# apache/spark

Measured on AMD Instinct MI355X. Metric: rows/sec (sort+hash-agg+join, 1B-row synth), higher is better.
Workload: dtype int64; 1 GPU; orderby-1b-int64x3 (BASELINE configs[1]); value = sort rows/s; rows=1000000000, cols=int64 key + int64 + float64 payload, parallelism=single GPU

## Files before the change

### spark_amd/csrc/gpuq.hip

```cpp
#include <hip/hip_runtime.h>
#include <stdint.h>
#include <stdio.h>
#include <string.h>

#include "../../include/gpuq.h"


static __thread char g_err[512];

extern "C" const char* gpuq_last_error(void) { return g_err; }

#define FAIL(code, ...) do { \
    snprintf(g_err, sizeof(g_err), __VA_ARGS__); return (code); } while (0)

#define HIP_TRY(expr) do { hipError_t _e = (expr); if (_e != hipSuccess) { \
    snprintf(g_err, sizeof(g_err), "%s failed: %s (%s:%d)", #expr, \
             hipGetErrorString(_e), __FILE__, __LINE__); \
    return GPUQ_ERR_HIP; } } while (0)

extern "C" int gpuq_device_count(void) {
  int n = 0;
  if (hipGetDeviceCount(&n) != hipSuccess) return 0;
  return n;
}
// ... 61 lines not shown
  h1 ^= k1; h1 = rotl32(h1, 13); return h1 * 5u + 0xe6546b64u;
}
DEV uint32_t mm3_fmix(uint32_t h1, uint32_t len) {
  h1 ^= len; h1 ^= h1 >> 16; h1 *= 0x85ebca6bu; h1 ^= h1 >> 13;
  h1 *= 0xc2b2ae35u; h1 ^= h1 >> 16; return h1;
}
DEV int32_t mm3_hash_long(int64_t input, int32_t seed) {
  uint32_t lo = (uint32_t)(uint64_t)input;
  uint32_t hi = (uint32_t)((uint64_t)input >> 32);
  uint32_t h1 = mm3_mixH1((uint32_t)seed, mm3_mixK1(lo));
  h1 = mm3_mixH1(h1, mm3_mixK1(hi));
  return (int32_t)mm3_fmix(h1, 8);
}
DEV int32_t spark_pmod(int32_t a, int32_t n) {
  int32_t r = a % n; return r < 0 ? r + n : r;
}

DEV uint64_t splitmix64(uint64_t x) {
  x += 0x9E3779B97F4A7C15ULL;
  x = (x ^ (x >> 30)) * 0xBF58476D1CE4E5B9ULL;
  x = (x ^ (x >> 27)) * 0x94D049BB133111EBULL;
  return x ^ (x >> 31);
}
DEV uint64_t gen_u64_dev(uint64_t seed, uint64_t i) {
  return splitmix64(seed * 0x9E3779B97F4A7C15ULL + i);
}

#define SIGNBIT 0x8000000000000000ULL

DEV uint64_t encode_f64(double v) {
  if (v == -0.0) v = 0.0;
  uint64_t bits;
  if (v != v) bits = 0x7ff8000000000000ULL;
  else bits = __double_as_longlong(v);
  uint64_t mask = (uint64_t)(-(int64_t)(bits >> 63)) | SIGNBIT;
  return bits ^ mask;
}
DEV uint64_t encode_i64(int64_t v) { return (uint64_t)v ^ SIGNBIT; }

DEV int64_t decode_i64(uint64_t e) { return (int64_t)(e ^ SIGNBIT); }
DEV double decode_f64(uint64_t e) {
  uint64_t mask = ((e >> 63) ? 0 : ~0ULL) | SIGNBIT;
  return __longlong_as_double((long long)(e ^ mask));
}

DEV uint64_t sort_out_word(uint64_t kk, int decode_mode) {
  if (!decode_mode) return kk;
  uint64_t e = (decode_mode & 4) ? ~kk : kk;
  if (decode_mode & 2) {
    uint64_t mask = ((e >> 63) ? 0 : ~0ULL) | SIGNBIT;
    return e ^ mask;
  }
  return e ^ SIGNBIT;
}

DEV bool bit_valid(const uint8_t* validity, int64_t i) {
  return !validity || ((validity[i >> 3] >> (i & 7)) & 1);
}


__global__ void k_gen_i64_range(uint64_t seed, uint64_t start, int64_t n,
                                uint64_t range, int64_t* out) {
  int64_t i = (int64_t)blockIdx.x * blockDim.x + threadIdx.x;
  int64_t stride = (int64_t)gridDim.x * blockDim.x;
  for (; i < n; i += stride) {
    uint64_t v = gen_u64_dev(seed, start + (uint64_t)i);
    out[i] = (int64_t)(range ? v % range : v);
  }
}

__global__ void k_gen_f64_unit(uint64_t seed, uint64_t start, int64_t n, double* out) {
  int64_t i = (int64_t)blockIdx.x * blockDim.x + threadIdx.x;
  int64_t stride = (int64_t)gridDim.x * blockDim.x;
  for (; i < n; i += stride) {
    uint64_t v = gen_u64_dev(seed, start + (uint64_t)i);
    out[i] = (double)(v >> 11) * (1.0 / 9007199254740992.0);
  }
}

static dim3 hash_grid(int64_t n, int block = 256) {
  static int cap = -2;
  if (cap == -2) {
    const char* e = getenv("GPUQ_HASH_GRID");
    cap = e ? atoi(e) : 2048;
  }
  int64_t b = (n + block - 1) / block;
  if (cap > 0 && b > cap) b = cap;
  if (b > 0x7FFFFFFF) b = 0x7FFFFFFF;
  if (b < 1) b = 1;
  return dim3((uint32_t)b);
}

static dim3 grid1d(int64_t n, int block = 256) {
  int64_t b = (n + block - 1) / block;
  if (b > 2048) b = 2048;
  if (b < 1) b = 1;
  return dim3((uint32_t)b);
}

extern "C" int gpuq_gen_i64_range(void* stream, uint64_t seed, uint64_t start,
                                  int64_t n, uint64_t range, int64_t* out) {
  k_gen_i64_range<<<grid1d(n), 256, 0, (hipStream_t)stream>>>(seed, start, n, range, out);
  HIP_TRY(hipGetLastError());
  return GPUQ_OK;
}

// ... 135 lines not shown
  if (n == 0) return GPUQ_OK;
  { hipEvent_t _pe = prof_begin(s);
  k_interleave2<<<grid1d(n), 256, 0, s>>>(n, (const uint64_t*)a,
                                          (const uint64_t*)b,
                                          (ulonglong2*)scratch);
  prof_end("interleave2", s, _pe); }
  HIP_TRY(hipGetLastError());
  static int mlp = -1;
  if (mlp < 0) mlp = getenv("GPUQ_GATHER_MLP") ? atoi(getenv("GPUQ_GATHER_MLP")) : 0;
  { hipEvent_t _pe = prof_begin(s);
  if (mlp)
    k_gather2_pairs4<<<grid1d((n + 3) / 4), 256, 0, s>>>(
        n, (const ulonglong2*)scratch, perm, (uint64_t*)oa, (uint64_t*)ob);
  else
    k_gather2_pairs<<<grid1d(n), 256, 0, s>>>(n, (const ulonglong2*)scratch,
                                              perm, (uint64_t*)oa,
                                              (uint64_t*)ob);
  prof_end("gather2_pairs", s, _pe); }
  HIP_TRY(hipGetLastError());
  return GPUQ_OK;
}

extern "C" int gpuq_gather(void* stream, int64_t n, gpuq_col col,
                           const uint32_t* perm, void* out) {
  hipStream_t s = (hipStream_t)stream;
  if (col.dtype == GPUQ_INT64 || col.dtype == GPUQ_FLOAT64) {
    k_gather<uint64_t><<<grid1d(n, 256), 256, 0, s>>>(n, (const uint64_t*)col.data, perm, (uint64_t*)out);
  } else if (col.dtype == GPUQ_INT32) {
    k_gather<uint32_t><<<grid1d(n, 256), 256, 0, s>>>(n, (const uint32_t*)col.data, perm, (uint32_t*)out);
  } else {
    FAIL(GPUQ_ERR_INVALID, "gather: unsupported dtype %d", col.dtype);
  }
  HIP_TRY(hipGetLastError());
  return GPUQ_OK;
}


#define SORT_BLOCK 256
#define SORT_WAVES (SORT_BLOCK / WAVE)
#define SORT_ITEMS 16
#define SORT_TILE (SORT_BLOCK * SORT_ITEMS)

template <int DTYPE, bool DESC>
__global__ void k_encode(int64_t n, const void* keys, const uint32_t* rowmap,
                         uint64_t* ek, uint32_t* idx,
                         unsigned long long* bits_and, unsigned long long* bits_or,
                         uint32_t* ghist ) {
  __shared__ uint32_t h[8][256];
  for (int b = threadIdx.x; b < 8 * 256; b += blockDim.x) ((uint32_t*)h)[b] = 0;
  __syncthreads();
  uint64_t acc_or = 0, acc_and = ~0ULL;
  int64_t i = (int64_t)blockIdx.x * blockDim.x + threadIdx.x;
  int64_t stride = (int64_t)gridDim.x * blockDim.x;
  for (; i < n; i += stride) {
    uint64_t e;
    uint32_t row = rowmap ? rowmap[i] : (uint32_t)i;
    if (DTYPE == GPUQ_FLOAT64) e = encode_f64(((const double*)keys)[row]);
    else e = encode_i64(((const int64_t*)keys)[row]);
    if (DESC) e = ~e;
    ek[i] = e;
    idx[i] = row;
    acc_or |= e; acc_and &= e;
    #pragma unroll
    for (int b = 0; b < 8; b++) atomicAdd(&h[b][(e >> (b * 8)) & 0xff], 1u);
  }
  for (int off = 32; off > 0; off >>= 1) {
    acc_or |= __shfl_down((unsigned long long)acc_or, off);
    acc_and &= __shfl_down((unsigned long long)acc_and, off);
  }
  if ((threadIdx.x & (WAVE - 1)) == 0) {
    atomicOr(bits_or, (unsigned long long)acc_or);
    atomicAnd(bits_and, (unsigned long long)acc_and);
  }
  __syncthreads();
  for (int b = threadIdx.x; b < 8 * 256; b += blockDim.x) {
    uint32_t v = ((uint32_t*)h)[b];
    if (v) atomicAdd(&ghist[b], v);
  }
}

struct scatter_geom { int block, items; };
static scatter_geom get_sort_geom(void);

template <int BIN_MODE>
DEV int compute_bin(uint64_t key, int shift, int nparts) {
  (void)nparts;
  if (BIN_MODE == 0) return (int)((key >> shift) & 0xff);
  if (BIN_MODE == 2)
    return (int)(((uint32_t)mm3_hash_long((int64_t)key, 42)) >> 24);
  return (int)((((uint32_t)mm3_hash_long((int64_t)key, 42)) >> (16 + shift)) & 0xff);
}

__global__ void k_validity_pids(int64_t n, const uint8_t* validity, int nulls_first,
                                uint64_t* pid_as_key, uint32_t* idx,
                                unsigned long long* null_count) {
  __shared__ unsigned int h;
  if (threadIdx.x == 0) h = 0;
  __syncthreads();
  int64_t i = (int64_t)blockIdx.x * blockDim.x + threadIdx.x;
  int64_t stride = (int64_t)gridDim.x * blockDim.x;
  unsigned int mine = 0;
  for (; i < n; i += stride) {
    bool valid = (validity[i >> 3] >> (i & 7)) & 1;
    pid_as_key[i] = (uint64_t)(valid == (bool)nulls_first);
    idx[i] = (uint32_t)i;
    if (!valid) mine++;
  }
  if (mine) atomicAdd(&h, mine);
  __syncthreads();
  if (threadIdx.x == 0 && h) atomicAdd(null_count, (unsigned long long)h);
}

template <int BIN_MODE>
__global__ void k_radix_hist(int64_t n, const uint64_t* keys, int shift,
// ... 65 lines not shown
    __syncthreads();
    if (threadIdx.x == 0) {
      uint32_t acc = 0;
      for (int w = 0; w < SCAN_BLOCK / WAVE; w++) { uint32_t t = wsum[w]; wsum[w] = acc; acc += t; }
      carry_s = acc;
    }
    __syncthreads();
    if (i < n) sums[i] = s - v + wsum[wave] + carry;
    carry += carry_s;
    __syncthreads();
  }
}

__global__ void k_scan_add(int64_t n, const uint32_t* in, uint32_t* out,
                           const uint32_t* block_sums) {
  int64_t base = (int64_t)blockIdx.x * SCAN_TILE;
  uint32_t add = block_sums[blockIdx.x];
  for (int r = 0; r < SCAN_ITEMS; r++) {
    int64_t i = base + r * SCAN_BLOCK + threadIdx.x;
    if (i < n) out[i] = out[i] - in[i] + add;
  }
}

static int exclusive_scan_u32(hipStream_t s, int64_t n, const uint32_t* in,
                              uint32_t* out, uint32_t* block_sums ) {
  int64_t nblocks = (n + SCAN_TILE - 1) / SCAN_TILE;
  k_scan_partial<<<dim3((uint32_t)nblocks), SCAN_BLOCK, 0, s>>>(n, in, out, block_sums);
  k_scan_sums<<<1, SCAN_BLOCK, 0, s>>>(nblocks, block_sums);
  k_scan_add<<<dim3((uint32_t)nblocks), SCAN_BLOCK, 0, s>>>(n, in, out, block_sums);
  HIP_TRY(hipGetLastError());
  return GPUQ_OK;
}

#define OSW_AGG (1ULL << 54)
#define OSW_PFX (2ULL << 54)
#define OSW_VAL(x) ((x) & ((1ULL << 54) - 1))
#define OSW_EPOCH(x) ((x) >> 56)
#define OSW_SPIN_LIMIT (1u << 22)

typedef unsigned long long ull2_a8 __attribute__((vector_size(16), aligned(8)));
typedef uint32_t u32v2_a4 __attribute__((vector_size(8), aligned(4)));

template <int BIN_MODE, int BLOCK, int ITEMS, bool LOOKBACK, typename PayT = uint32_t,
          int RADIX_BITS = 8, bool CONTIG = false>
__global__ __launch_bounds__(BLOCK)
void k_radix_scatter(int64_t n, const uint64_t* kin, const PayT* iin,
                     uint64_t* kout, PayT* iout,
                     const uint32_t* scanned ,
                     int shift, int nblocks, int nparts,
                     unsigned long long* state ,
                     const uint32_t* gbase ,
                     unsigned long long* err_flag, uint32_t epoch,
                     void* decode_out ,
                     int decode_mode ) {
  constexpr int WAVES = BLOCK / WAVE;
  constexpr int TILE = BLOCK * ITEMS;
  constexpr int BINS = 1 << RADIX_BITS;
  __shared__ uint32_t wave_hist[WAVES][BINS];
  __shared__ uint32_t bin_start[BINS];
  __shared__ uint32_t bin_gbase[BINS];
  __shared__ uint32_t wtot[WAVES <= 4 ? 4 : WAVES];
  __shared__ uint32_t bin_cnt[(LOOKBACK && RADIX_BITS < 8) ? BINS : 1];
  __shared__ uint64_t stage_k[TILE];
  __shared__ PayT stage_i[TILE];

  const int tid = threadIdx.x;
  const int wave = tid / WAVE, lane = tid & (WAVE - 1);
  const int64_t base = (int64_t)blockIdx.x * TILE;
  const int tile_n = (int)min((int64_t)TILE, n - base);

  for (int b = tid; b < WAVES * BINS; b += BLOCK)
    ((uint32_t*)wave_hist)[b] = 0;
  __syncthreads();

  uint64_t k[ITEMS];
  PayT id[ITEMS];
  uint16_t lrank[ITEMS];
  uint8_t lbin[ITEMS];

  const int64_t wbase = base + (int64_t)wave * WAVE * ITEMS;
  #pragma unroll
  for (int r = 0; r < ITEMS; r++) {
    int64_t i = wbase + r * WAVE + lane;
    bool valid = i < n;
    k[r] = valid ? kin[i] : 0;
    id[r] = valid ? iin[i] : 0;
  }
  for (int r = 0; r < ITEMS; r++) {
    int64_t i = wbase + r * WAVE + lane;
    bool valid = i < n;
    int bin = valid ? compute_bin<BIN_MODE>(k[r], shift, nparts) : 0;
    if (RADIX_BITS < 8) bin &= (1 << RADIX_BITS) - 1;
    lbin[r] = (uint8_t)bin;
    uint64_t active = __ballot(valid);
    uint64_t same = active;
    for (int b = 0; b < RADIX_BITS; b++) {
      uint64_t bl = __ballot((bin >> b) & 1);
      same &= ((bin >> b) & 1) ? bl : ~bl;
    }
    uint64_t below = same & ((1ULL << lane) - 1);
    int rank = __popcll(below);
    int leader = __ffsll((unsigned long long)same) - 1;
    uint32_t basecnt = 0;
    if (valid && lane == leader) {
      basecnt = wave_hist[wave][bin];
      wave_hist[wave][bin] = basecnt + __popcll(same);
    }
    basecnt = __shfl(basecnt, leader);
    lrank[r] = (uint16_t)(basecnt + rank);
    __builtin_amdgcn_wave_barrier();
  }
  __syncthreads();

  uint32_t acc = 0;
  if (tid < BINS) {
    int bin = tid;
    for (int w = 0; w < WAVES; w++) {
      uint32_t t = wave_hist[w][bin];
      wave_hist[w][bin] = acc;
      acc += t;
    }
    if (LOOKBACK) {
      __hip_atomic_store(&state[(int64_t)blockIdx.x * 256 + bin],
                         ((unsigned long long)epoch << 56) | OSW_AGG | acc,
                         __ATOMIC_RELAXED, __HIP_MEMORY_SCOPE_AGENT);
      if (RADIX_BITS < 8) bin_cnt[bin] = acc;
    }
    uint32_t inc = wave_inclusive_scan(acc);
    if (lane == WAVE - 1) wtot[wave] = inc;
    bin_start[bin] = inc - acc;
  }
  __syncthreads();
  if (tid < BINS) {
    int bin = tid;
    uint32_t woff = 0;
    for (int w = 0; w < wave; w++) woff += wtot[w];
    uint32_t excl = bin_start[bin] + woff;
    bin_start[bin] = excl;
    if (!LOOKBACK) {
// ... 152 lines not shown
    if (j < tile_n) {
      uint64_t kk = stage_k[j];
      int bin = compute_bin<BIN_MODE>(kk, shift, nparts);
      if (RADIX_BITS < 8) bin &= (1 << RADIX_BITS) - 1;
      uint32_t dst = bin_gbase[bin] + (uint32_t)j;
      uint64_t kv_out = sort_out_word(kk, decode_mode);
      void* kdst = decode_mode ? (void*)&((uint64_t*)decode_out)[dst]
                               : (void*)&kout[dst];
#ifdef GPUQ_DRAIN_SC1
      __hip_atomic_store((uint64_t*)kdst, kv_out, __ATOMIC_RELAXED,
                         __HIP_MEMORY_SCOPE_AGENT);
      __hip_atomic_store((PayT*)&iout[dst], stage_i[j], __ATOMIC_RELAXED,
                         __HIP_MEMORY_SCOPE_AGENT);
#elif defined(GPUQ_DRAIN_NT)
      __builtin_nontemporal_store(kv_out, (uint64_t*)kdst);
      __builtin_nontemporal_store(stage_i[j], &iout[dst]);
#else
      *(uint64_t*)kdst = kv_out;
      iout[dst] = stage_i[j];
#endif
    }
  }
}

static scatter_geom get_sort_geom(void) {
  static scatter_geom g = {0, 0};
  if (g.block == 0) {
    const char* e = getenv("GPUQ_SORT_GEOM");
    int b = 0, it = 0;
    if (e && sscanf(e, "%dx%d", &b, &it) == 2) { g.block = b; g.items = it; }
    else { g.block = 256; g.items = 22; }
    static const int known[][2] = {{256,16},{512,8},{512,16},{1024,8},{512,4},
                                   {512,6},{256,12},{512,12},{1024,5},{512,10},
                                   {1024,2},{1024,6},{1024,4},{512,11},
                                   {256,20},{256,22}};
    bool ok = false;
    for (auto& k : known) ok = ok || (k[0] == g.block && k[1] == g.items);
    if (!ok) {
      fprintf(stderr, "gpuq: unsupported GPUQ_SORT_GEOM %dx%d, using 256x22\n",
              g.block, g.items);
      g.block = 256; g.items = 22;
    }
  }
  return g;
}

template <int BIN_MODE, bool LOOKBACK>
static void launch_scatter(hipStream_t s, scatter_geom g, int64_t nb,
                           int64_t n, const uint64_t* kin, const uint32_t* iin,
                           uint64_t* kout, uint32_t* iout,
                           const uint32_t* scanned, int shift, int nparts,
                           unsigned long long* state, const uint32_t* gbase,
                           unsigned long long* err_flag, uint32_t epoch,
                           void* decode_out = nullptr, int decode_mode = 0) {
  dim3 grid((uint32_t)nb);
#define LS(B, I) k_radix_scatter<BIN_MODE, B, I, LOOKBACK><<<grid, B, 0, s>>>( \
      n, kin, iin, kout, iout, scanned, shift, (int)nb, nparts, state, gbase, \
      err_flag, epoch, decode_out, decode_mode)
  static int contig = -1;
  if (contig < 0) contig = getenv("GPUQ_DRAIN_CONTIG") != nullptr;
  if (contig && g.block == 512 && (g.items == 9 || g.items == 10 || g.items == 11)) {
    if (g.items == 9)
      k_radix_scatter<BIN_MODE, 512, 9, LOOKBACK, uint32_t, 8, true><<<grid, 512, 0, s>>>(
          n, kin, iin, kout, iout, scanned, shift, (int)nb, nparts, state, gbase,
          err_flag, epoch, decode_out, decode_mode);
    else if (g.items == 11)
      k_radix_scatter<BIN_MODE, 512, 11, LOOKBACK, uint32_t, 8, true><<<grid, 512, 0, s>>>(
          n, kin, iin, kout, iout, scanned, shift, (int)nb, nparts, state, gbase,
          err_flag, epoch, decode_out, decode_mode);
    else
      k_radix_scatter<BIN_MODE, 512, 10, LOOKBACK, uint32_t, 8, true><<<grid, 512, 0, s>>>(
          n, kin, iin, kout, iout, scanned, shift, (int)nb, nparts, state, gbase,
          err_flag, epoch, decode_out, decode_mode);
    return;
  }
  if (g.block == 256 && g.items == 20)
    k_radix_scatter<BIN_MODE, 256, 20, LOOKBACK><<<grid, 256, 0, s>>>(
      n, kin, iin, kout, iout, scanned, shift, (int)nb, nparts, state, gbase,
      err_flag, epoch, decode_out, decode_mode);
  else if (g.block == 256 && g.items == 22)
    k_radix_scatter<BIN_MODE, 256, 22, LOOKBACK><<<grid, 256, 0, s>>>(
      n, kin, iin, kout, iout, scanned, shift, (int)nb, nparts, state, gbase,
      err_flag, epoch, decode_out, decode_mode);
  else if (g.block == 512 && g.items == 11)
    k_radix_scatter<BIN_MODE, 512, 11, LOOKBACK><<<grid, 512, 0, s>>>(
      n, kin, iin, kout, iout, scanned, shift, (int)nb, nparts, state, gbase,
      err_flag, epoch, decode_out, decode_mode);
  else if (g.block == 256 && g.items == 16) LS(256, 16);
  else if (g.block == 512 && g.items == 8) LS(512, 8);
  else if (g.block == 512 && g.items == 16) LS(512, 16);
  else if (g.block == 1024 && g.items == 8) LS(1024, 8);
  else if (g.block == 512 && g.items == 4) LS(512, 4);
  else if (g.block == 512 && g.items == 6)
    k_radix_scatter<BIN_MODE, 512, 6, LOOKBACK><<<grid, 512, 0, s>>>(
      n, kin, iin, kout, iout, scanned, shift, (int)nb, nparts, state, gbase,
      err_flag, epoch, decode_out, decode_mode);
  else if (g.block == 256 && g.items == 12)
    k_radix_scatter<BIN_MODE, 256, 12, LOOKBACK><<<grid, 256, 0, s>>>(
      n, kin, iin, kout, iout, scanned, shift, (int)nb, nparts, state, gbase,
      err_flag, epoch, decode_out, decode_mode);
  else if (g.block == 512 && g.items == 12)
    k_radix_scatter<BIN_MODE, 512, 12, LOOKBACK><<<grid, 512, 0, s>>>(
      n, kin, iin, kout, iout, scanned, shift, (int)nb, nparts, state, gbase,
      err_flag, epoch, decode_out, decode_mode);
  else if (g.block == 1024 && g.items == 5)
    k_radix_scatter<BIN_MODE, 1024, 5, LOOKBACK><<<grid, 1024, 0, s>>>(
      n, kin, iin, kout, iout, scanned, shift, (int)nb, nparts, state, gbase,
      err_flag, epoch, decode_out, decode_mode);
  else if (g.block == 512 && g.items == 10)
    k_radix_scatter<BIN_MODE, 512, 10, LOOKBACK><<<grid, 512, 0, s>>>(
      n, kin, iin, kout, iout, scanned, shift, (int)nb, nparts, state, gbase,
      err_flag, epoch, decode_out, decode_mode);
  else if (g.block == 1024 && g.items == 2) LS(1024, 2);
  else if (g.block == 1024 && g.items == 6) LS(1024, 6);
  else LS(1024, 4);
#undef LS
}

template <int MODE>
__global__ __launch_bounds__(512)
void k_scatter_ablate(int64_t n, const uint64_t* kin, const uint32_t* iin,
                      uint64_t* kout, uint32_t* iout,
                      const uint32_t* gbase, unsigned long long* sink,
                      int shift) {
  constexpr int BLOCK = 512, ITEMS = 10, WAVES = BLOCK / WAVE;
  constexpr int TILE = BLOCK * ITEMS;
  __shared__ uint32_t wave_hist[WAVES][256];
  __shared__ uint32_t bin_start[256];
  __shared__ uint32_t bin_gbase[256];
  __shared__ uint32_t wtot[WAVES < 4 ? 4 : WAVES];
  __shared__ uint64_t stage_k[TILE];
  __shared__ uint32_t stage_i[TILE];
  const int tid = threadIdx.x;
  const int wave = tid / WAVE, lane = tid & (WAVE - 1);
  const int64_t base = (int64_t)blockIdx.x * TILE;
  const int tile_n = (int)min((int64_t)TILE, n - base);
  for (int b = tid; b < WAVES * 256; b += BLOCK) ((uint32_t*)wave_hist)[b] = 0;
  __syncthreads();
  uint64_t k[ITEMS]; uint32_t id[ITEMS]; uint16_t lrank[ITEMS]; uint8_t lbin[ITEMS];
  const int64_t wbase = base + (int64_t)wave * WAVE * ITEMS;
  #pragma unroll
  for (int r = 0; r < ITEMS; r++) {
    int64_t i = wbase + r * WAVE + lane;
    bool valid = i < n;
    k[r] = valid ? kin[i] : 0;
    id[r] = valid ? iin[i] : 0;
  }
  if (MODE == 0) {
    uint64_t acc = 0;
    for (int r = 0; r < ITEMS; r++) acc ^= k[r] + id[r];
    if (acc == 0xDEADBEEFCAFEBABEull) atomicAdd(sink, 1ull);
    return;
  }
  for (int r = 0; r < ITEMS; r++) {
    int64_t i = wbase + r * WAVE + lane;
    bool valid = i < n;
    int bin = valid ? (int)((k[r] >> shift) & 0xff) : 0;
    lbin[r] = (uint8_t)bin;
    uint64_t m = __ballot(valid);
    for (int b = 0; b < 8; b++) {
      uint64_t bl = __ballot((bin >> b) & 1);
      m &= ((bin >> b) & 1) ? bl : ~bl;
    }
    uint64_t below = m & ((1ULL << lane) - 1);
    int rank = __popcll(below);
// ... 157 lines not shown
        rec.x = (uint32_t)kk; rec.y = (uint32_t)(kk >> 32);
        rec.z = stage_i[j]; rec.w = 0;
        ((uint4*)rout)[dst] = rec;
      }
    }
  }
}

extern "C" int gpuq_scatter_ablate2(void* stream, int64_t n, const void* kin,
                                    const void* iin, void* kout, void* iout,
                                    void* rout, const void* gbase, int32_t mode) {
  hipStream_t s = (hipStream_t)stream;
  int64_t nb = (n + 4095) / 4096;
  if (mode == 4)
    k_scatter_ablate2<4><<<dim3((uint32_t)nb), 512, 0, s>>>(
        n, (const uint64_t*)kin, (const uint32_t*)iin, (uint64_t*)kout,
        (uint32_t*)iout, (uint32_t*)rout, (const uint32_t*)gbase, 0);
  else
    k_scatter_ablate2<5><<<dim3((uint32_t)nb), 512, 0, s>>>(
        n, (const uint64_t*)kin, (const uint32_t*)iin, (uint64_t*)kout,
        (uint32_t*)iout, (uint32_t*)rout, (const uint32_t*)gbase, 0);
  HIP_TRY(hipGetLastError());
  return GPUQ_OK;
}

extern "C" int gpuq_scatter_ablate(void* stream, int64_t n, const void* kin,
                                   const void* iin, void* kout, void* iout,
                                   const void* gbase, void* sink, int32_t mode) {
  hipStream_t s = (hipStream_t)stream;
  int64_t nb = (n + 5119) / 5120;
  dim3 g((uint32_t)nb);
#define AB(M) k_scatter_ablate<M><<<g, 512, 0, s>>>(n, (const uint64_t*)kin, \
    (const uint32_t*)iin, (uint64_t*)kout, (uint32_t*)iout, \
    (const uint32_t*)gbase, (unsigned long long*)sink, 0)
  if (mode == 0) AB(0); else if (mode == 1) AB(1);
  else if (mode == 2) AB(2); else AB(3);
#undef AB
  HIP_TRY(hipGetLastError());
  return GPUQ_OK;
}

template <int BIN_MODE, bool LOOKBACK>
static void launch_scatter4(hipStream_t s, scatter_geom g, int64_t nb,
                            int64_t n, const uint64_t* kin, const uint32_t* iin,
                            uint64_t* kout, uint32_t* iout,
                            const uint32_t* scanned, int shift, int nparts,
                            unsigned long long* state, const uint32_t* gbase,
                            unsigned long long* err_flag, uint32_t epoch,
                            void* decode_out = nullptr, int decode_mode = 0) {
  dim3 grid((uint32_t)nb);
  if (g.block == 1024 && g.items == 8)
    k_radix_scatter<BIN_MODE, 1024, 8, LOOKBACK, uint32_t, 4><<<grid, 1024, 0, s>>>(
        n, kin, iin, kout, iout, scanned, shift, (int)nb, nparts, state, gbase,
        err_flag, epoch, decode_out, decode_mode);
  else if (g.block == 256 && g.items == 22)
    k_radix_scatter<BIN_MODE, 256, 22, LOOKBACK, uint32_t, 4><<<grid, 256, 0, s>>>(
        n, kin, iin, kout, iout, scanned, shift, (int)nb, nparts, state, gbase,
        err_flag, epoch, decode_out, decode_mode);
  else if (g.block == 512 && g.items == 10)
    k_radix_scatter<BIN_MODE, 512, 10, LOOKBACK, uint32_t, 4><<<grid, 512, 0, s>>>(
        n, kin, iin, kout, iout, scanned, shift, (int)nb, nparts, state, gbase,
        err_flag, epoch, decode_out, decode_mode);
  else
    k_radix_scatter<BIN_MODE, 512, 10, LOOKBACK, uint32_t, 4><<<grid, 512, 0, s>>>(
        n, kin, iin, kout, iout, scanned, shift, (int)nb, nparts, state, gbase,
        err_flag, epoch, decode_out, decode_mode);
}

template <int DTYPE, bool DESC>
__global__ void k_decode(int64_t n, const uint64_t* ek, void* out) {
  int64_t i = (int64_t)blockIdx.x * blockDim.x + threadIdx.x;
  int64_t stride = (int64_t)gridDim.x * blockDim.x;
  for (; i < n; i += stride) {
    uint64_t e = ek[i];
    if (DESC) e = ~e;
    if (DTYPE == GPUQ_FLOAT64) {
      uint64_t mask = ((e >> 63) ? 0 : ~0ULL) | SIGNBIT;
      ((uint64_t*)out)[i] = e ^ mask;
    } else {
      ((int64_t*)out)[i] = (int64_t)(e ^ SIGNBIT);
    }
  }
}

#define GPUQ_SORT_TIE_MAX 32
#define TIEFIX_BLOCK 256
#define TIEFIX_ITEMS 8
#define TIEFIX_TILE (TIEFIX_BLOCK * TIEFIX_ITEMS)

__global__ __launch_bounds__(TIEFIX_BLOCK)
void k_sort_tiefix(int64_t n, const uint64_t* kin, const uint32_t* iin,
                   uint32_t* out_perm, uint64_t* out_keys ,
                   int shift, int decode_mode, unsigned long long* overflow) {
  constexpr int HALO = GPUQ_SORT_TIE_MAX;
  __shared__ uint64_t tk[TIEFIX_TILE + 2 * HALO];
  const int tid = threadIdx.x;
  const int64_t base = (int64_t)blockIdx.x * TIEFIX_TILE;
  uint32_t id[TIEFIX_ITEMS];
  #pragma unroll
  for (int r = 0; r < TIEFIX_ITEMS; r++) {
    int64_t i = base + r * TIEFIX_BLOCK + tid;
    id[r] = i < n ? iin[i] : 0;
  }
  for (int j = tid; j < TIEFIX_TILE + 2 * HALO; j += TIEFIX_BLOCK) {
    int64_t g = base - HALO + j;
    tk[j] = (g >= 0 && g < n) ? kin[g] : 0;
  }
  __syncthreads();
  #pragma unroll
  for (int r = 0; r < TIEFIX_ITEMS; r++) {
    const int j = r * TIEFIX_BLOCK + tid;
    const int64_t i = base + j;
    if (i >= n) break;
    const uint64_t* c = &tk[HALO + j];
    const uint64_t k = c[0];
    const uint64_t win = k >> shift;
    int back = 0, fwd = 0;
    while (back < HALO && i - back - 1 >= 0 && (c[-back - 1] >> shift) == win) back++;
    while (fwd < HALO && i + fwd + 1 < n && (c[fwd + 1] >> shift) == win) fwd++;
// ... 55 lines not shown
extern "C" void gpuq_sort_last_plan(int* window_passes, int* deferred_bytes,
                                    int* fell_back) {
  if (window_passes) *window_passes = g_sort_plan.window_passes;
  if (deferred_bytes) *deferred_bytes = g_sort_plan.deferred_bytes;
  if (fell_back) *fell_back = g_sort_plan.fell_back;
}

struct sort_ws {
  uint64_t* ka; uint64_t* kb;
  uint32_t* ia; uint32_t* ib;
  uint32_t* hist; uint32_t* hist_scan; uint32_t* block_sums;
  unsigned long long* bits;
  uint32_t* ghist;
  uint32_t* gbase;
  unsigned long long* state;
  unsigned long long* err;
};

static int64_t sort_nblocks(int64_t n, int tile) { return (n + tile - 1) / tile; }

static void sort_ws_layout(int64_t n, int nbins, sort_ws* w, char* basep, int64_t* total) {
  int tile = get_sort_geom().block * get_sort_geom().items;
  int64_t nb = sort_nblocks(n, tile);
  int64_t hist_n = (int64_t)nbins * nb;
  int64_t scan_blocks = (hist_n + SCAN_TILE - 1) / SCAN_TILE + 1;
  int64_t off = 0;
  auto take = [&](int64_t bytes) {
    char* p = basep ? basep + off : nullptr;
    off += (bytes + 255) & ~255LL;
    return p;
  };
  w->ka = (uint64_t*)take(n * 8);
  w->kb = (uint64_t*)take(n * 8);
  w->ia = (uint32_t*)take(n * 4);
  w->ib = (uint32_t*)take(n * 4);
  w->hist = (uint32_t*)take(hist_n * 4);
  w->hist_scan = (uint32_t*)take(hist_n * 4);
  w->block_sums = (uint32_t*)take(scan_blocks * 4);
  w->bits = (unsigned long long*)take(16);
  w->ghist = (uint32_t*)take(8 * 256 * 4);
  w->gbase = (uint32_t*)take(8 * 256 * 4);
  w->state = (unsigned long long*)take(nb * 256 * 8);
  w->err = (unsigned long long*)take(16);
  *total = off;
}

extern "C" int64_t gpuq_sort_workspace_bytes(int64_t n) {
  sort_ws w; int64_t total;
  sort_ws_layout(n, 256, &w, nullptr, &total);
  return total;
}

static void launch_encode(hipStream_t s, int64_t n, const void* keys,
                          const uint32_t* rowmap, int dtype, int desc, sort_ws* w) {
  if (dtype == GPUQ_FLOAT64) {
    if (desc) k_encode<GPUQ_FLOAT64, true><<<grid1d(n), 256, 0, s>>>(n, keys, rowmap, w->ka, w->ia, &w->bits[0], &w->bits[1], w->ghist);
    else      k_encode<GPUQ_FLOAT64, false><<<grid1d(n), 256, 0, s>>>(n, keys, rowmap, w->ka, w->ia, &w->bits[0], &w->bits[1], w->ghist);
  } else {
    if (desc) k_encode<GPUQ_INT64, true><<<grid1d(n), 256, 0, s>>>(n, keys, rowmap, w->ka, w->ia, &w->bits[0], &w->bits[1], w->ghist);
    else      k_encode<GPUQ_INT64, false><<<grid1d(n), 256, 0, s>>>(n, keys, rowmap, w->ka, w->ia, &w->bits[0], &w->bits[1], w->ghist);
  }
}

extern "C" int gpuq_sort_perm(void* stream, int64_t n, gpuq_col key,
                              int32_t desc, int32_t nulls_first,
                              uint32_t* out_perm, void* out_keys,
                              void* workspace, int64_t workspace_bytes) {
  hipStream_t s = (hipStream_t)stream;
  if (n > 0xFFFFFFFFLL) FAIL(GPUQ_ERR_INVALID, "sort: nrows %lld > 2^32", (long long)n);
  if (key.dtype != GPUQ_INT64 && key.dtype != GPUQ_FLOAT64)
    FAIL(GPUQ_ERR_INVALID, "sort: unsupported dtype %d", key.dtype);
  sort_ws w; int64_t need;
  sort_ws_layout(n, 256, &w, (char*)workspace, &need);
  if (workspace_bytes < need)
    FAIL(GPUQ_ERR_INVALID, "sort: workspace %lld < %lld", (long long)workspace_bytes, (long long)need);
  if (n == 0) return GPUQ_OK;

  scatter_geom geom = get_sort_geom();
  int tile = geom.block * geom.items;
  static __thread int force_classic = 0;
  static __thread int force_no_prefix = 0;
  bool onesweep = !force_classic && getenv("GPUQ_NO_ONESWEEP") == nullptr;
  bool no_prefix = force_no_prefix || getenv("GPUQ_SORT_NO_PREFIX") != nullptr;
  g_sort_plan = sort_plan_rec{0, 0, 0};

  int64_t n_sort = n;
  int64_t sorted_at = 0;
  const uint32_t* rowmap = nullptr;
  if (key.validity) {
    int64_t nbv = sort_nblocks(n, tile);
    HIP_TRY(hipMemsetAsync(w.err, 0, 8, s));
    k_validity_pids<<<grid1d(n), 256, 0, s>>>(n, key.validity, nulls_first,
                                              w.ka, w.ia, w.err);
    HIP_TRY(hipGetLastError());
    k_radix_hist<0><<<dim3((uint32_t)nbv), 256, 0, s>>>(n, w.ka, 0, w.hist, (int)nbv, tile);
    HIP_TRY(hipGetLastError());
    int rc = exclusive_scan_u32(s, 256 * nbv, w.hist, w.hist_scan, w.block_sums);
    if (rc) return rc;
    launch_scatter<0, false>(s, geom, nbv, n, w.ka, w.ia, w.kb, w.ib, w.hist_scan,
                             0, 0, nullptr, nullptr, nullptr, 0);
    HIP_TRY(hipGetLastError());
    unsigned long long hnull = 0;
    HIP_TRY(hipMemcpyAsync(&hnull, w.err, 8, hipMemcpyDeviceToHost, s));
    HIP_TRY(hipStreamSynchronize(s));
    int64_t nnull = (int64_t)hnull;
    n_sort = n - nnull;
    sorted_at = nulls_first ? nnull : 0;
    int64_t nulls_at_out = nulls_first ? 0 : n_sort;
    int64_t nulls_at_ib = nulls_first ? 0 : n_sort;
    if (nnull > 0)
      HIP_TRY(hipMemcpyAsync(out_perm + nulls_at_out, w.ib + nulls_at_ib,
                             nnull * 4, hipMemcpyDeviceToDevice, s));
    rowmap = w.ib + sorted_at;
    if (n_sort == 0) {
      if (out_keys) {
        gpuq_col kc = key; kc.validity = nullptr;
        return gpuq_gather(stream, n, kc, out_perm, out_keys);
      }
      return GPUQ_OK;
    }
  }

  int64_t nb = sort_nblocks(n_sort, tile);
  HIP_TRY(hipMemsetAsync(w.bits, 0, 16, s));
  HIP_TRY(hipMemsetAsync(w.bits, 0xFF, 8, s));
  HIP_TRY(hipMemsetAsync(w.ghist, 0, 8 * 256 * 4, s));
  { hipEvent_t _pe = prof_begin(s);
  launch_encode(s, n_sort, key.data, rowmap, key.dtype, desc, &w);
  prof_end("encode", s, _pe); }
  HIP_TRY(hipGetLastError());
  unsigned long long hb[2];
  uint32_t hghist[8 * 256];
  HIP_TRY(hipMemcpyAsync(hb, w.bits, 16, hipMemcpyDeviceToHost, s));
  HIP_TRY(hipMemcpyAsync(hghist, w.ghist, sizeof(hghist), hipMemcpyDeviceToHost, s));
  HIP_TRY(hipStreamSynchronize(s));
  uint64_t bits_changed = hb[0] ^ hb[1];

  bool nibble_mode = onesweep && getenv("GPUQ_SORT_BITS") != nullptr &&
                     atoi(getenv("GPUQ_SORT_BITS")) == 4;
  if (nibble_mode && !((geom.block == 1024 && geom.items == 8) ||
                       (geom.block == 512 && geom.items == 10) ||
                       (geom.block == 256 && geom.items == 22)))
    nibble_mode = false;
  int retries = 0;
retry:
  int prefix_low = -1;
  if (!nibble_mode && !no_prefix) {
    int wp = 0, db = 0;
    prefix_low = sort_prefix_plan(bits_changed, hghist, n_sort, &wp, &db);
    if (prefix_low >= 0) g_sort_plan = sort_plan_rec{wp, db, 0};
  }
  if (onesweep && !nibble_mode) {
    uint32_t hgbase[8 * 256];
    for (int b = 0; b < 8; b++) {
      uint32_t run = 0;
      for (int bin = 0; bin < 256; bin++) {
        hgbase[b * 256 + bin] = run;
        run += hghist[b * 256 + bin];
      }
    }
    HIP_TRY(hipMemcpyAsync(w.gbase, hgbase, sizeof(hgbase), hipMemcpyHostToDevice, s));
    HIP_TRY(hipMemsetAsync(w.state, 0, nb * 256 * 8, s));
    HIP_TRY(hipMemsetAsync(w.err, 0, 16, s));
  } else if (nibble_mode) {
    uint32_t hgbase[16 * 16];
    for (int lvl = 0; lvl < 16; lvl++) {
      int byte = lvl / 2;
      bool high = lvl & 1;
      uint32_t cnt[16] = {0};
      for (int v = 0; v < 256; v++) {
        int nib = high ? (v >> 4) : (v & 15);
        cnt[nib] += hghist[byte * 256 + v];
      }
      uint32_t run = 0;
      for (int v = 0; v < 16; v++) { hgbase[lvl * 16 + v] = run; run += cnt[v]; }
    }
    HIP_TRY(hipMemcpyAsync(w.gbase, hgbase, sizeof(hgbase), hipMemcpyHostToDevice, s));
    HIP_TRY(hipMemsetAsync(w.state, 0, nb * 256 * 8, s));
    HIP_TRY(hipMemsetAsync(w.err, 0, 16, s));
  } else if (prefix_low >= 0) {
    HIP_TRY(hipMemsetAsync(w.err, 0, 16, s));
  }

  int nlevels = nibble_mode ? 16 : 8;
  int lvl_bits = nibble_mode ? 4 : 8;
  uint64_t lvl_mask = nibble_mode ? 0xfULL : 0xffULL;
  int last_byte = -1;
  for (int lvl = 0; lvl < nlevels; lvl++)
    if (((bits_changed >> (lvl * lvl_bits)) & lvl_mask) != 0) last_byte = lvl;
  uint64_t *kin = w.ka, *kout = w.kb;
  uint32_t *iin = w.ia, *iout = w.ib;
  for (int byte = 0; byte < nlevels; byte++) {
    if (((bits_changed >> (byte * lvl_bits)) & lvl_mask) == 0) continue;
    if (byte < prefix_low) continue;
    int shift = byte * lvl_bits;
    bool final_pass = byte == last_byte && prefix_low < 0;
    uint32_t* iout_pass = final_pass ? out_perm + sorted_at : iout;
    void* dec_out = nullptr;
    int dec_mode = 0;
    if (final_pass && out_keys && !key.validity) {
      dec_out = (char*)out_keys;
      dec_mode = (key.dtype == GPUQ_FLOAT64 ? 2 : 1) | (desc ? 4 : 0);
    }
    if (nibble_mode) {
      { hipEvent_t _pe = prof_begin(s);
      launch_scatter4<0, true>(s, geom, nb, n_sort, kin, iin, kout, iout_pass, nullptr,
                               shift, 0, w.state, w.gbase + byte * 16, w.err,
                               (uint32_t)(byte + 1), dec_out, dec_mode);
      prof_end("radix_scatter", s, _pe); }
      HIP_TRY(hipGetLastError());
    } else if (onesweep) {
      { hipEvent_t _pe = prof_begin(s);
      launch_scatter<0, true>(s, geom, nb, n_sort, kin, iin, kout, iout_pass, nullptr,
                              shift, 0, w.state, w.gbase + byte * 256, w.err,
                              (uint32_t)(byte + 1), dec_out, dec_mode);
      prof_end("radix_scatter", s, _pe); }
      HIP_TRY(hipGetLastError());
    } else {
      { hipEvent_t _pe = prof_begin(s);
      k_radix_hist<0><<<dim3((uint32_t)nb), 256, 0, s>>>(n_sort, kin, shift, w.hist, (int)nb, tile);
      prof_end("radix_hist", s, _pe); }
      HIP_TRY(hipGetLastError());
      int rc = exclusive_scan_u32(s, (int64_t)256 * nb, w.hist, w.hist_scan, w.block_sums);
      if (rc) return rc;
      { hipEvent_t _pe = prof_begin(s);
      launch_scatter<0, false>(s, geom, nb, n_sort, kin, iin, kout, iout_pass, w.hist_scan,
                               shift, 0, nullptr, nullptr, nullptr, 0, dec_out, dec_mode);
      prof_end("radix_scatter", s, _pe); }
      HIP_TRY(hipGetLastError());
    }
    uint64_t* tk = kin; kin = kout; kout = tk;
    uint32_t* ti = iin; iin = iout_pass; iout = ti;
  }

  if (prefix_low >= 0) {
    void* kdst = (out_keys && !key.validity) ? out_keys : nullptr;
    int dec_mode = (key.dtype == GPUQ_FLOAT64 ? 2 : 1) | (desc ? 4 : 0);
    { hipEvent_t _pe = prof_begin(s);
    k_sort_tiefix<<<dim3((uint32_t)sort_nblocks(n_sort, TIEFIX_TILE)), TIEFIX_BLOCK, 0, s>>>(
        n_sort, kin, iin, out_perm + sorted_at, (uint64_t*)kdst, prefix_low * 8,
        dec_mode, &w.err[1]);
    prof_end("sort_tiefix", s, _pe); }
    HIP_TRY(hipGetLastError());
  }

  if (onesweep || prefix_low >= 0) {
    unsigned long long herr2[2] = {0, 0};
    HIP_TRY(hipMemcpyAsync(herr2, w.err, 16, hipMemcpyDeviceToHost, s));
    HIP_TRY(hipStreamSynchronize(s));
    unsigned long long herr = onesweep ? herr2[0] : 0;
    if (!herr && prefix_low >= 0 && herr2[1]) {
      g_sort_plan.fell_back = 1;
      no_prefix = true;
      if (key.validity) {
        sort_plan_rec tried = g_sort_plan;
        force_no_prefix = 1;
        int rc = gpuq_sort_perm(stream, n, key, desc, nulls_first, out_perm,
                                out_keys, workspace, workspace_bytes);
        force_no_prefix = 0;
        g_sort_plan = tried;
        return rc;
      }
      launch_encode(s, n_sort, key.data, nullptr, key.dtype, desc, &w);
      HIP_TRY(hipGetLastError());
      goto retry;
    }
    if (herr) {
      if (++retries > 1) FAIL(GPUQ_ERR_HIP, "sort: lookback timed out twice");
      onesweep = false;
      if (key.validity) {
        force_classic = 1;
        int rc = gpuq_sort_perm(stream, n, key, desc, nulls_first, out_perm,
                                out_keys, workspace, workspace_bytes);
        force_classic = 0;
        return rc;
      }
      launch_encode(s, n_sort, key.data, nullptr, key.dtype, desc, &w);
      HIP_TRY(hipGetLastError());
      goto retry;
    }
  }
  if (last_byte < 0)
    HIP_TRY(hipMemcpyAsync(out_perm + sorted_at, iin, n_sort * 4, hipMemcpyDeviceToDevice, s));
  if (out_keys) {
    if (key.validity) {
      gpuq_col kc = key; kc.validity = nullptr;
      int rc = gpuq_gather(stream, n, kc, out_perm, out_keys);
      if (rc) return rc;
    } else if (last_byte >= 0) {
    } else {
      if (key.dtype == GPUQ_FLOAT64) {
        if (desc) k_decode<GPUQ_FLOAT64, true><<<grid1d(n), 256, 0, s>>>(n, kin, out_keys);
        else      k_decode<GPUQ_FLOAT64, false><<<grid1d(n), 256, 0, s>>>(n, kin, out_keys);
      } else {
        if (desc) k_decode<GPUQ_INT64, true><<<grid1d(n), 256, 0, s>>>(n, kin, out_keys);
        else      k_decode<GPUQ_INT64, false><<<grid1d(n), 256, 0, s>>>(n, kin, out_keys);
      }
      HIP_TRY(hipGetLastError());
    }
  }
  return GPUQ_OK;
}



__global__ void k_partition_pids(int64_t n, const int64_t* keys, const uint8_t* validity,
                                 int32_t nparts, uint64_t* pid_as_key, uint32_t* idx,
                                 unsigned long long* counts ) {
  __shared__ uint32_t h[256];
  bool lds_counts = nparts <= 256;
  if (lds_counts)
    for (int b = threadIdx.x; b < nparts; b += blockDim.x) h[b] = 0;
  __syncthreads();
  int64_t i = (int64_t)blockIdx.x * blockDim.x + threadIdx.x;
  int64_t stride = (int64_t)gridDim.x * blockDim.x;
  for (; i < n; i += stride) {
    int32_t hsh = 42;
    if (bit_valid(validity, i)) hsh = mm3_hash_long(keys[i], 42);
    int pid = spark_pmod(hsh, nparts);
    pid_as_key[i] = (uint64_t)pid;
    idx[i] = (uint32_t)i;
    if (lds_counts) atomicAdd(&h[pid], 1u);
    else atomicAdd(&counts[pid], 1ull);
  }
  __syncthreads();
  if (lds_counts)
    for (int b = threadIdx.x; b < nparts; b += blockDim.x)
      if (h[b]) atomicAdd(&counts[b], (unsigned long long)h[b]);
}
// ... 2707 lines not shown
```

Measured before the change: 13.74 billion rows/s.

## Fuse key encoding into first onesweep radix pass, make encode histogram-only

When onesweep is active and keys have no validity or aliasing, the encode kernel only computes the bit masks and digit histograms, without writing encoded keys and row indices. The first radix scatter pass then reads raw keys, encodes them in registers and generates identity indices itself. This removes a full write and re-read of 1B 64-bit keys plus 32-bit indices. The histogram-only loop is also unrolled 4x. It adds per-element encode work to the first scatter pass, and makes the fallback and retry paths more complex.

```diff
diff --git a/spark_amd/csrc/gpuq.hip b/spark_amd/csrc/gpuq.hip
--- a/spark_amd/csrc/gpuq.hip
+++ b/spark_amd/csrc/gpuq.hip
@@ -137,6 +137,13 @@
     return e ^ mask;
   }
   return e ^ SIGNBIT;
+}
+
+DEV uint64_t sort_in_word(uint64_t raw, int in_mode) {
+  if (!in_mode) return raw;
+  uint64_t e = (in_mode & 2) ? encode_f64(__longlong_as_double((long long)raw))
+                             : encode_i64((int64_t)raw);
+  return (in_mode & 4) ? ~e : e;
 }
 
 DEV bool bit_valid(const uint8_t* validity, int64_t i) {
@@ -378,14 +385,33 @@
   uint64_t acc_or = 0, acc_and = ~0ULL;
   int64_t i = (int64_t)blockIdx.x * blockDim.x + threadIdx.x;
   int64_t stride = (int64_t)gridDim.x * blockDim.x;
+  if (!ek) {
+    for (; i + 3 * stride < n; i += 4 * stride) {
+      uint64_t e[4];
+      #pragma unroll
+      for (int u = 0; u < 4; u++) {
+        if (DTYPE == GPUQ_FLOAT64) e[u] = encode_f64(((const double*)keys)[i + u * stride]);
+        else e[u] = encode_i64(((const int64_t*)keys)[i + u * stride]);
+        if (DESC) e[u] = ~e[u];
+      }
+      #pragma unroll
+      for (int u = 0; u < 4; u++) {
+        acc_or |= e[u]; acc_and &= e[u];
+        #pragma unroll
+        for (int b = 0; b < 8; b++) atomicAdd(&h[b][(e[u] >> (b * 8)) & 0xff], 1u);
+      }
+    }
+  }
   for (; i < n; i += stride) {
     uint64_t e;
     uint32_t row = rowmap ? rowmap[i] : (uint32_t)i;
     if (DTYPE == GPUQ_FLOAT64) e = encode_f64(((const double*)keys)[row]);
     else e = encode_i64(((const int64_t*)keys)[row]);
     if (DESC) e = ~e;
-    ek[i] = e;
-    idx[i] = row;
+    if (ek) {
+      ek[i] = e;
+      idx[i] = row;
+    }
     acc_or |= e; acc_and &= e;
     #pragma unroll
     for (int b = 0; b < 8; b++) atomicAdd(&h[b][(e >> (b * 8)) & 0xff], 1u);
@@ -557,7 +583,8 @@
                      const uint32_t* gbase ,
                      unsigned long long* err_flag, uint32_t epoch,
                      void* decode_out ,
-                     int decode_mode ) {
+                     int decode_mode ,
+                     int in_mode ) {
   constexpr int WAVES = BLOCK / WAVE;
   constexpr int TILE = BLOCK * ITEMS;
   constexpr int BINS = 1 << RADIX_BITS;
@@ -584,12 +611,25 @@
   uint8_t lbin[ITEMS];
 
   const int64_t wbase = base + (int64_t)wave * WAVE * ITEMS;
-  #pragma unroll
-  for (int r = 0; r < ITEMS; r++) {
-    int64_t i = wbase + r * WAVE + lane;
-    bool valid = i < n;
-    k[r] = valid ? kin[i] : 0;
-    id[r] = valid ? iin[i] : 0;
+  if (iin) {
+    #pragma unroll
+    for (int r = 0; r < ITEMS; r++) {
+      int64_t i = wbase + r * WAVE + lane;
+      bool valid = i < n;
+      k[r] = valid ? kin[i] : 0;
+      id[r] = valid ? iin[i] : 0;
+    }
+  } else {
+    #pragma unroll
+    for (int r = 0; r < ITEMS; r++) {
+      int64_t i = wbase + r * WAVE + lane;
+      k[r] = i < n ? kin[i] : 0;
+      id[r] = (PayT)i;
+    }
+  }
+  if (in_mode) {
+    #pragma unroll
+    for (int r = 0; r < ITEMS; r++) k[r] = sort_in_word(k[r], in_mode);
   }
   for (int r = 0; r < ITEMS; r++) {
     int64_t i = wbase + r * WAVE + lane;
@@ -848,40 +888,41 @@
                            const uint32_t* scanned, int shift, int nparts,
                            unsigned long long* state, const uint32_t* gbase,
                            unsigned long long* err_flag, uint32_t epoch,
-                           void* decode_out = nullptr, int decode_mode = 0) {
+                           void* decode_out = nullptr, int decode_mode = 0,
+                           int in_mode = 0) {
   dim3 grid((uint32_t)nb);
 #define LS(B, I) k_radix_scatter<BIN_MODE, B, I, LOOKBACK><<<grid, B, 0, s>>>( \
       n, kin, iin, kout, iout, scanned, shift, (int)nb, nparts, state, gbase, \
-      err_flag, epoch, decode_out, decode_mode)
+      err_flag, epoch, decode_out, decode_mode, in_mode)
   static int contig = -1;
   if (contig < 0) contig = getenv("GPUQ_DRAIN_CONTIG") != nullptr;
   if (contig && g.block == 512 && (g.items == 9 || g.items == 10 || g.items == 11)) {
     if (g.items == 9)
       k_radix_scatter<BIN_MODE, 512, 9, LOOKBACK, uint32_t, 8, true><<<grid, 512, 0, s>>>(
           n, kin, iin, kout, iout, scanned, shift, (int)nb, nparts, state, gbase,
-          err_flag, epoch, decode_out, decode_mode);
+          err_flag, epoch, decode_out, decode_mode, in_mode);
     else if (g.items == 11)
       k_radix_scatter<BIN_MODE, 512, 11, LOOKBACK, uint32_t, 8, true><<<grid, 512, 0, s>>>(
           n, kin, iin, kout, iout, scanned, shift, (int)nb, nparts, state, gbase,
-          err_flag, epoch, decode_out, decode_mode);
+          err_flag, epoch, decode_out, decode_mode, in_mode);
     else
       k_radix_scatter<BIN_MODE, 512, 10, LOOKBACK, uint32_t, 8, true><<<grid, 512, 0, s>>>(
           n, kin, iin, kout, iout, scanned, shift, (int)nb, nparts, state, gbase,
-          err_flag, epoch, decode_out, decode_mode);
+          err_flag, epoch, decode_out, decode_mode, in_mode);
     return;
   }
   if (g.block == 256 && g.items == 20)
     k_radix_scatter<BIN_MODE, 256, 20, LOOKBACK><<<grid, 256, 0, s>>>(
       n, kin, iin, kout, iout, scanned, shift, (int)nb, nparts, state, gbase,
-      err_flag, epoch, decode_out, decode_mode);
+      err_flag, epoch, decode_out, decode_mode, in_mode);
   else if (g.block == 256 && g.items == 22)
     k_radix_scatter<BIN_MODE, 256, 22, LOOKBACK><<<grid, 256, 0, s>>>(
       n, kin, iin, kout, iout, scanned, shift, (int)nb, nparts, state, gbase,
-      err_flag, epoch, decode_out, decode_mode);
+      err_flag, epoch, decode_out, decode_mode, in_mode);
   else if (g.block == 512 && g.items == 11)
     k_radix_scatter<BIN_MODE, 512, 11, LOOKBACK><<<grid, 512, 0, s>>>(
       n, kin, iin, kout, iout, scanned, shift, (int)nb, nparts, state, gbase,
-      err_flag, epoch, decode_out, decode_mode);
+      err_flag, epoch, decode_out, decode_mode, in_mode);
   else if (g.block == 256 && g.items == 16) LS(256, 16);
   else if (g.block == 512 && g.items == 8) LS(512, 8);
   else if (g.block == 512 && g.items == 16) LS(512, 16);
@@ -890,23 +931,23 @@
   else if (g.block == 512 && g.items == 6)
     k_radix_scatter<BIN_MODE, 512, 6, LOOKBACK><<<grid, 512, 0, s>>>(
       n, kin, iin, kout, iout, scanned, shift, (int)nb, nparts, state, gbase,
-      err_flag, epoch, decode_out, decode_mode);
+      err_flag, epoch, decode_out, decode_mode, in_mode);
   else if (g.block == 256 && g.items == 12)
     k_radix_scatter<BIN_MODE, 256, 12, LOOKBACK><<<grid, 256, 0, s>>>(
       n, kin, iin, kout, iout, scanned, shift, (int)nb, nparts, state, gbase,
-      err_flag, epoch, decode_out, decode_mode);
+      err_flag, epoch, decode_out, decode_mode, in_mode);
   else if (g.block == 512 && g.items == 12)
     k_radix_scatter<BIN_MODE, 512, 12, LOOKBACK><<<grid, 512, 0, s>>>(
       n, kin, iin, kout, iout, scanned, shift, (int)nb, nparts, state, gbase,
-      err_flag, epoch, decode_out, decode_mode);
+      err_flag, epoch, decode_out, decode_mode, in_mode);
   else if (g.block == 1024 && g.items == 5)
     k_radix_scatter<BIN_MODE, 1024, 5, LOOKBACK><<<grid, 1024, 0, s>>>(
       n, kin, iin, kout, iout, scanned, shift, (int)nb, nparts, state, gbase,
-      err_flag, epoch, decode_out, decode_mode);
+      err_flag, epoch, decode_out, decode_mode, in_mode);
   else if (g.block == 512 && g.items == 10)
     k_radix_scatter<BIN_MODE, 512, 10, LOOKBACK><<<grid, 512, 0, s>>>(
       n, kin, iin, kout, iout, scanned, shift, (int)nb, nparts, state, gbase,
-      err_flag, epoch, decode_out, decode_mode);
+      err_flag, epoch, decode_out, decode_mode, in_mode);
   else if (g.block == 1024 && g.items == 2) LS(1024, 2);
   else if (g.block == 1024 && g.items == 6) LS(1024, 6);
   else LS(1024, 4);
@@ -1170,19 +1211,19 @@
   if (g.block == 1024 && g.items == 8)
     k_radix_scatter<BIN_MODE, 1024, 8, LOOKBACK, uint32_t, 4><<<grid, 1024, 0, s>>>(
         n, kin, iin, kout, iout, scanned, shift, (int)nb, nparts, state, gbase,
-        err_flag, epoch, decode_out, decode_mode);
+        err_flag, epoch, decode_out, decode_mode, 0 );
   else if (g.block == 256 && g.items == 22)
     k_radix_scatter<BIN_MODE, 256, 22, LOOKBACK, uint32_t, 4><<<grid, 256, 0, s>>>(
         n, kin, iin, kout, iout, scanned, shift, (int)nb, nparts, state, gbase,
-        err_flag, epoch, decode_out, decode_mode);
+        err_flag, epoch, decode_out, decode_mode, 0 );
   else if (g.block == 512 && g.items == 10)
     k_radix_scatter<BIN_MODE, 512, 10, LOOKBACK, uint32_t, 4><<<grid, 512, 0, s>>>(
         n, kin, iin, kout, iout, scanned, shift, (int)nb, nparts, state, gbase,
-        err_flag, epoch, decode_out, decode_mode);
+        err_flag, epoch, decode_out, decode_mode, 0 );
   else
     k_radix_scatter<BIN_MODE, 512, 10, LOOKBACK, uint32_t, 4><<<grid, 512, 0, s>>>(
         n, kin, iin, kout, iout, scanned, shift, (int)nb, nparts, state, gbase,
-        err_flag, epoch, decode_out, decode_mode);
+        err_flag, epoch, decode_out, decode_mode, 0 );
 }
 
 template <int DTYPE, bool DESC>
@@ -1344,13 +1385,16 @@
 }
 
 static void launch_encode(hipStream_t s, int64_t n, const void* keys,
-                          const uint32_t* rowmap, int dtype, int desc, sort_ws* w) {
+                          const uint32_t* rowmap, int dtype, int desc, sort_ws* w,
+                          bool hist_only = false) {
+  uint64_t* ek = hist_only ? nullptr : w->ka;
+  uint32_t* idx = hist_only ? nullptr : w->ia;
   if (dtype == GPUQ_FLOAT64) {
-    if (desc) k_encode<GPUQ_FLOAT64, true><<<grid1d(n), 256, 0, s>>>(n, keys, rowmap, w->ka, w->ia, &w->bits[0], &w->bits[1], w->ghist);
-    else      k_encode<GPUQ_FLOAT64, false><<<grid1d(n), 256, 0, s>>>(n, keys, rowmap, w->ka, w->ia, &w->bits[0], &w->bits[1], w->ghist);
+    if (desc) k_encode<GPUQ_FLOAT64, true><<<grid1d(n), 256, 0, s>>>(n, keys, rowmap, ek, idx, &w->bits[0], &w->bits[1], w->ghist);
+    else      k_encode<GPUQ_FLOAT64, false><<<grid1d(n), 256, 0, s>>>(n, keys, rowmap, ek, idx, &w->bits[0], &w->bits[1], w->ghist);
   } else {
-    if (desc) k_encode<GPUQ_INT64, true><<<grid1d(n), 256, 0, s>>>(n, keys, rowmap, w->ka, w->ia, &w->bits[0], &w->bits[1], w->ghist);
-    else      k_encode<GPUQ_INT64, false><<<grid1d(n), 256, 0, s>>>(n, keys, rowmap, w->ka, w->ia, &w->bits[0], &w->bits[1], w->ghist);
+    if (desc) k_encode<GPUQ_INT64, true><<<grid1d(n), 256, 0, s>>>(n, keys, rowmap, ek, idx, &w->bits[0], &w->bits[1], w->ghist);
+    else      k_encode<GPUQ_INT64, false><<<grid1d(n), 256, 0, s>>>(n, keys, rowmap, ek, idx, &w->bits[0], &w->bits[1], w->ghist);
   }
 }
 
@@ -1417,9 +1461,21 @@
   HIP_TRY(hipMemsetAsync(w.bits, 0, 16, s));
   HIP_TRY(hipMemsetAsync(w.bits, 0xFF, 8, s));
   HIP_TRY(hipMemsetAsync(w.ghist, 0, 8 * 256 * 4, s));
+  bool nibble_mode = onesweep && getenv("GPUQ_SORT_BITS") != nullptr &&
+                     atoi(getenv("GPUQ_SORT_BITS")) == 4;
+  if (nibble_mode && !((geom.block == 1024 && geom.items == 8) ||
+                       (geom.block == 512 && geom.items == 10) ||
+                       (geom.block == 256 && geom.items == 22)))
+    nibble_mode = false;
+  const char* kraw = (const char*)key.data;
+  bool keys_alias = out_keys && (const char*)out_keys < kraw + n * 8 &&
+                    kraw < (const char*)out_keys + n * 8;
+  bool fused = onesweep && !nibble_mode && !key.validity && !keys_alias &&
+               getenv("GPUQ_SORT_NO_FUSED_ENCODE") == nullptr;
+  const int key_mode = (key.dtype == GPUQ_FLOAT64 ? 2 : 1) | (desc ? 4 : 0);
   { hipEvent_t _pe = prof_begin(s);
-  launch_encode(s, n_sort, key.data, rowmap, key.dtype, desc, &w);
-  prof_end("encode", s, _pe); }
+  launch_encode(s, n_sort, key.data, rowmap, key.dtype, desc, &w, fused);
+  prof_end(fused ? "sort_hist" : "encode", s, _pe); }
   HIP_TRY(hipGetLastError());
   unsigned long long hb[2];
   uint32_t hghist[8 * 256];
@@ -1427,13 +1483,13 @@
   HIP_TRY(hipMemcpyAsync(hghist, w.ghist, sizeof(hghist), hipMemcpyDeviceToHost, s));
   HIP_TRY(hipStreamSynchronize(s));
   uint64_t bits_changed = hb[0] ^ hb[1];
-
-  bool nibble_mode = onesweep && getenv("GPUQ_SORT_BITS") != nullptr &&
-                     atoi(getenv("GPUQ_SORT_BITS")) == 4;
-  if (nibble_mode && !((geom.block == 1024 && geom.items == 8) ||
-                       (geom.block == 512 && geom.items == 10) ||
-                       (geom.block == 256 && geom.items == 22)))
-    nibble_mode = false;
+  if (fused && bits_changed == 0) {
+    fused = false;
+    { hipEvent_t _pe = prof_begin(s);
+    launch_encode(s, n_sort, key.data, nullptr, key.dtype, desc, &w);
+    prof_end("encode", s, _pe); }
+    HIP_TRY(hipGetLastError());
+  }
   int retries = 0;
 retry:
   int prefix_low = -1;
@@ -1480,8 +1536,11 @@
   int last_byte = -1;
   for (int lvl = 0; lvl < nlevels; lvl++)
     if (((bits_changed >> (lvl * lvl_bits)) & lvl_mask) != 0) last_byte = lvl;
-  uint64_t *kin = w.ka, *kout = w.kb;
-  uint32_t *iin = w.ia, *iout = w.ib;
+  const uint64_t* kin = fused ? (const uint64_t*)key.data : w.ka;
+  const uint32_t* iin = fused ? nullptr : w.ia;
+  uint64_t *kout = w.kb, *knext = w.ka;
+  uint32_t *iout = w.ib, *inext = w.ia;
+  int in_mode = fused ? key_mode : 0;
   for (int byte = 0; byte < nlevels; byte++) {
     if (((bits_changed >> (byte * lvl_bits)) & lvl_mask) == 0) continue;
     if (byte < prefix_low) continue;
@@ -1505,7 +1564,7 @@
       { hipEvent_t _pe = prof_begin(s);
       launch_scatter<0, true>(s, geom, nb, n_sort, kin, iin, kout, iout_pass, nullptr,
                               shift, 0, w.state, w.gbase + byte * 256, w.err,
-                              (uint32_t)(byte + 1), dec_out, dec_mode);
+                              (uint32_t)(byte + 1), dec_out, dec_mode, in_mode);
       prof_end("radix_scatter", s, _pe); }
       HIP_TRY(hipGetLastError());
     } else {
@@ -1521,8 +1580,9 @@
       prof_end("radix_scatter", s, _pe); }
       HIP_TRY(hipGetLastError());
     }
-    uint64_t* tk = kin; kin = kout; kout = tk;
-    uint32_t* ti = iin; iin = iout_pass; iout = ti;
+    uint64_t* kdone = kout; kout = knext; knext = kdone; kin = kdone;
+    uint32_t* idone = iout; iout = inext; inext = idone; iin = iout_pass;
+    in_mode = 0;
   }
 
   if (prefix_low >= 0) {
@@ -1553,8 +1613,10 @@
         g_sort_plan = tried;
         return rc;
       }
-      launch_encode(s, n_sort, key.data, nullptr, key.dtype, desc, &w);
-      HIP_TRY(hipGetLastError());
+      if (!fused) {
+        launch_encode(s, n_sort, key.data, nullptr, key.dtype, desc, &w);
+        HIP_TRY(hipGetLastError());
+      }
       goto retry;
     }
     if (herr) {
@@ -1567,6 +1629,7 @@
         force_classic = 0;
         return rc;
       }
+      fused = false;
       launch_encode(s, n_sort, key.data, nullptr, key.dtype, desc, &w);
       HIP_TRY(hipGetLastError());
       goto retry;
```

Result: faster. 14.33 billion rows/s, median of 6 (+4.3%).
